# fabiocarrara/neural-ode-features

Measured on AMD Instinct MI355X. Metric: images/sec (fwd+adjoint) CIFAR-10 ODE-ResNet bs=128 at 1/2/4/8 GPU, higher is better.
Workload: dtype f32

## Files before the change

### neural-ode-features_amd/csrc/kernels_pointwise.hip

```cpp
#include "node_internal.h"
#include "wino4.h"
#include "step_control.h"
#include <cstring>
#include "../../include/node_hip.h"

namespace node {


__device__ inline float wave_sum(float v) {
#pragma unroll
  for (int off = 32; off > 0; off >>= 1) v += __shfl_xor(v, off, 64);
  return v;
}
__device__ inline float wave_max(float v) {
#pragma unroll
  for (int off = 32; off > 0; off >>= 1) v = fmaxf(v, __shfl_xor(v, off, 64));
  return v;
}

__device__ inline float block_sum_256(float v, float* red ) {
  v = wave_sum(v);
  __syncthreads();
  if ((threadIdx.x & 63) == 0) red[threadIdx.x >> 6] = v;
  __syncthreads();
// ... 801 lines not shown
}
void launch_fill(float* p, float v, size_t n, hipStream_t s) {
  size_t blocks = (n + 255) / 256;
  if (blocks > 2048) blocks = 2048;
  if (blocks == 0) return;
  hipLaunchKernelGGL(k_fill, dim3((unsigned)blocks), dim3(256), 0, s, p, v, n);
}

__global__ __launch_bounds__(256) void k_dot_partial(const float* a, const float* b, size_t n, float* partial) {
  __shared__ float red[4];
  float acc = 0.f;
  const size_t stride = (size_t)gridDim.x * 256;
  for (size_t i = (size_t)blockIdx.x * 256 + threadIdx.x; i < n; i += stride) acc += a[i] * b[i];
  const float tot = block_sum_256(acc, red);
  if (threadIdx.x == 0) partial[blockIdx.x] = tot;
}
__global__ __launch_bounds__(256) void k_dot_final(Ctrl* c, const float* partial, float sign, float* out_dot) {
  __shared__ float red[4];
  const float tot = sign * reduce_partials_512(partial, red);
  if (threadIdx.x == 0) {
    c->ts_cur = c->ts_cur - tot;
    if (out_dot) *out_dot = tot;
  }
}
void launch_dot_sub_scalar(Ctrl* ctrl, const float* a, const float* b, size_t n, float sign, float* partial, float* out_dot, hipStream_t s) {
  hipLaunchKernelGGL(k_dot_partial, dim3(ERR_BLOCKS), dim3(256), 0, s, a, b, n, partial);
  hipLaunchKernelGGL(k_dot_final, dim3(1), dim3(256), 0, s, ctrl, partial, sign, out_dot);
}
__global__ void k_copy_scalar_out(const Ctrl* c, float* dst) { *dst = c->ts_cur; }
void launch_copy_scalar_out(const Ctrl* ctrl, float* dst, hipStream_t s) {
  hipLaunchKernelGGL(k_copy_scalar_out, dim3(1), dim3(1), 0, s, ctrl, dst);
}

__global__ __launch_bounds__(256) void k_theta_finalize(ThetaFinalizeArgs a, Dims d) {
  if (a.ctrl->done) return;
  __shared__ float red[256];
  __shared__ int s_last;
  const ThetaLayout L = theta_layout(d.C);
  const int C = d.C;
  const int nsm = (9 * C + 63) / 64;
  const int bx_all = blockIdx.x;
  const int wb = ((int)gridDim.x - 5 * nsm) / 2;
  if (bx_all >= 5 * nsm) {
    const int layer = (bx_all - 5 * nsm) / wb, bx = (bx_all - 5 * nsm) - layer * wb;
    const size_t CC = (size_t)C * C;
    const size_t n4 = 9 * CC / 4;
    const float4* wp = reinterpret_cast<const float4*>(a.wpart[layer]);
    float4* out = reinterpret_cast<float4*>(a.theta_out + L.wc[layer]);
    const size_t stride = (size_t)wb * 256;
    if (a.dU != nullptr) {
      const size_t cc4 = CC / 4;
      const float4* du = reinterpret_cast<const float4*>(a.dU + (size_t)layer * W4_COMPS * CC);
      for (size_t i = (size_t)bx * 256 + threadIdx.x; i < cc4; i += stride) {
        float4 tq[6][3];
#pragma unroll
        for (int xi = 0; xi < 6; ++xi) {
          float4 u[6];
#pragma unroll
          for (int nu = 0; nu < 6; ++nu) u[nu] = du[(size_t)(xi * 6 + nu) * cc4 + i];
#pragma unroll
          for (int kw = 0; kw < 3; ++kw) {
            float4 s = make_float4(0.f, 0.f, 0.f, 0.f);
#pragma unroll
            for (int nu = 0; nu < 6; ++nu) {
              const float gq = (float)W4_G[nu][kw];
              if (gq != 0.f) { s.x += gq * u[nu].x; s.y += gq * u[nu].y; s.z += gq * u[nu].z; s.w += gq * u[nu].w; }
            }
// ... 62 lines not shown
      a.theta_out[(which ? L.b[layer] : L.g[layer]) + (col - which * C)] = a.osign * v;
    }
    return;
  }
  if (on) {
    a.theta_out[L.wt[layer] + col] = a.osign * (v * eval_time(a.et));
    if (col >= 4 * C && col < 5 * C) a.theta_out[L.cb[layer] + (col - 4 * C)] = a.osign * v;
  }
  const int nb = (9 * C + 63) / 64;
  float* dotpart = a.sred + (size_t)2 * 9 * C;
  unsigned* counter = reinterpret_cast<unsigned*>(dotpart + 2 * nb);
  const float part = wave_sum(on ? v * a.wtime[layer][col] : 0.f);
#if defined(__HIP_DEVICE_COMPILE__) && !defined(__gfx950__)
#error "k_theta_finalize's fence-free hand-off is only valid on gfx950: use release/acquire on the counter elsewhere"
#endif
  if (cl == 0) {
    __hip_atomic_store(dotpart + layer * nb + bxs, part, __ATOMIC_RELAXED, __HIP_MEMORY_SCOPE_AGENT);
    asm volatile("s_waitcnt vmcnt(0)" ::: "memory");
    s_last = __hip_atomic_fetch_add(counter, 1u, __ATOMIC_RELAXED, __HIP_MEMORY_SCOPE_AGENT) == (unsigned)(2 * nb - 1);
  }
  __builtin_amdgcn_wave_barrier();
  if (!s_last) return;
  float tot = 0.f;
  for (int i = cl; i < 2 * nb; i += 64) tot += __hip_atomic_load(dotpart + i, __ATOMIC_RELAXED, __HIP_MEMORY_SCOPE_AGENT);
  tot = wave_sum(tot);
  if (cl == 0) {
    __hip_atomic_store(counter, 0u, __ATOMIC_RELAXED, __HIP_MEMORY_SCOPE_AGENT);
    if (a.write_scalar) a.ctrl->ts_k[a.kidx] = a.osign * tot;
    if (a.vjp_t_out) *a.vjp_t_out = a.osign * tot;
  }
}

void launch_theta_finalize(const Dims& d, const ThetaFinalizeArgs& a, hipStream_t s) {
  size_t wblocks = (9 * (size_t)d.C * d.C / 4 + 255) / 256;
  if (a.dU != nullptr) wblocks = ((size_t)d.C * d.C / 4 + 255) / 256;
  if (wblocks > 1024) wblocks = 1024;
  const size_t nsmall = (9 * (size_t)d.C + 63) / 64;
  hipLaunchKernelGGL(k_theta_finalize, dim3((unsigned)(5 * nsmall + 2 * wblocks)), dim3(256), 0, s, a, d);
}

__global__ __launch_bounds__(256) void k_lincomb(Comb c, const Ctrl* ctrl, float* out, size_t n) {
  const float scale = comb_scale(c, ctrl);
  float cf[7];
#pragma unroll
  for (int j = 0; j < 7; ++j) cf[j] = scale * c.coef[j];
  const size_t stride = (size_t)gridDim.x * 256;
  for (size_t i = (size_t)blockIdx.x * 256 + threadIdx.x; i < n; i += stride) {
    float s = 0.f;
    for (int j = 0; j < c.nk; ++j) s += cf[j] * c.k[j][i];
    out[i] = c.y[i] + s;
  }
}
void launch_lincomb(const Comb& c, const Ctrl* ctrl, float* out, size_t n, hipStream_t s) {
  size_t blocks = (n + 255) / 256;
  if (blocks > 2048) blocks = 2048;
  hipLaunchKernelGGL(k_lincomb, dim3((unsigned)blocks), dim3(256), 0, s, c, ctrl, out, n);
}

}
```

### neural-ode-features_amd/csrc/node_internal.h

```cpp
#pragma once
#include <hip/hip_runtime.h>
#include <stdint.h>
#include <stddef.h>

namespace node {

constexpr int KCH = 32;
constexpr int BN = 64;
constexpr int WG_THREADS = 256;

struct Dims {
  int N, C, H, W, HW, G, cpg;
  float eps;
  int Wp, Hp, SLOTS;
  int MARGIN;
  int BNE;
  int ntile;
  int nchunk;
  int BM;
  int S;
  int wino;
  int wgrad_wino;
  int wut;
  int tiny;
// ... 323 lines not shown
void launch_pack_weights_small(const Dims& d, const float* w, float* packed , hipStream_t s);
void launch_conv_small(const Dims& d, const ConvArgs& a, hipStream_t s);

struct WgradArgs {
  const float* act;
  const float* dz;
  const Ctrl* ctrl;
  float* wpart;
  unsigned long long* stamps;
  const float* act2;
  const float* dz2;
  float* wpart2;
};
void launch_wgrad(const Dims& d, const WgradArgs& a, hipStream_t s);
size_t wgrad_lds_bytes(const Dims& d);

struct ThetaFinalizeArgs {
  const float* dU;
  const float* wpart[2];
  const float* spart[2];
  const float* gpart[3];
  int gpart_rows[3];
  int spart_rows;
  const float* wtime[2];
  float* sred;
  EvalTime et;
  float osign;
  float* theta_out;
  Ctrl* ctrl;
  int kidx;
  int write_scalar;
  float* vjp_t_out;
};
void launch_theta_finalize(const Dims& d, const ThetaFinalizeArgs& a, hipStream_t s);

struct TinyConvArgs {
  const float* act;
  const unsigned short* wq;
  const float* bias; const float* tmap;
  EvalTime et;
  const float* gamma; const float* beta;
  float* out;
  float* part; unsigned* counter;
  const Ctrl* ctrl;
  int relu; float osign;
  int nx_on, nx_self;
  Comb nx; float* nx_y_out; const float* nx_gamma; const float* nx_beta; float* nx_act;
};
struct TinyResidentArgs {
  const float* y0;
  float* y_first;
  float* y_out;
  const float* w[2];
  const float* bias[2];
  const float* gamma[3];
  const float* beta[3];
  void* handoff;
  unsigned nonce;
  Ctrl* ctrl;
  Ctrl* ctrl_host;
  const double* targets; int n_targets;
  double targets_inline[8];
  const double* forced; int n_forced;
  double* dt_log; int dt_log_cap;
  double t0;
  long long max_steps;
  float rtol, atol, tsign;
// ... 36 lines not shown
```

### neural-ode-features_amd/csrc/plan.h

```cpp
#pragma once
#include "host_common.h"
#include "wino4.h"

namespace node {

struct Plan {
  Ctrl* ctrl;
  unsigned* arrive;
  float* partial[3];
  float* wf[2];
  float* wd[2];
  float* tmap[2];
  float *Y, *Y1, *KY[7];
  float *act1, *act2;
  float* RAW;
  float* wsmall[2];
  unsigned short* wtiny[2];
  float* tpart;
  unsigned* tcount;
  void* thand;
  float *W4V, *W4M;
  float* w4u[4];
  unsigned short* w4ub[4];
  float* tmapS[2];
  W4Scales* w4sc;
  float* W4Va0b;
  float *W4Va[2], *W4Z[2], *W4dU;
  float *act1b, *xh1b, *r1b;
  float *A, *A1, *KA[7];
  float *TH, *TH1, *KT[7];
  float *xh1, *xh2, *xh3, *r1, *r2, *r3;
  float *dz1, *dz2, *G;
  float *wpart[2], *spart[2], *gpart[3], *sred, *wtime[2];
  float* dots;
  double* targets;
  double* forced;
  double* dtlog;
  size_t bytes;
};
constexpr int STEP_LIST_CAP = 4096;

Plan make_plan(const Dims& d, int adjoint, int n_t, void* base);

int check_common(const node_shape* shape, const node_params* params, void* ws, size_t ws_bytes, int adjoint, int n_t,
                 Dims* d, Plan* plan);
int check_method(int method);
int check_times(const float* t_pts, int n_t);

struct SolveCtl {
  bool forced;
  int n_forced;
  long long max_steps;
  int log_cap;
  int blind;
};
int check_solve(const node_shape* shape, const node_params* params, void* ws, size_t ws_bytes, int adjoint, const float* t_pts,
                int n_t, int method, const node_solve_opts* opts, Dims* d, Plan* plan, SolveCtl* ctl);
int solve_rc(int status, double dt);

}
```

### neural-ode-features_amd/csrc/plan.hip

```cpp
#include "plan.h"

#include <cstring>

namespace node {

Plan make_plan(const Dims& d, int adjoint, int n_t, void* base) {
  Plan p;
  memset(&p, 0, sizeof(p));
  Bump b(base);
  p.ctrl = b.take<Ctrl>(1);
  p.arrive = b.take<unsigned>(4);
  p.targets = b.take<double>((size_t)(n_t > 0 ? n_t : 1));
  p.forced = b.take<double>(STEP_LIST_CAP);
  p.dtlog = b.take<double>(STEP_LIST_CAP);
  for (int i = 0; i < 3; ++i) p.partial[i] = b.take<float>(ERR_BLOCKS * 2);
  const size_t wsz = conv_packed_elems(d);
  for (int i = 0; i < 2; ++i) p.wf[i] = b.take<float>(wsz);
  for (int i = 0; i < 2; ++i) p.tmap[i] = b.take<float>((size_t)d.HW * d.C);
  p.Y = b.take<float>(d.numel);
  p.Y1 = b.take<float>(d.numel);
  for (int i = 0; i < 7; ++i) p.KY[i] = b.take<float>(d.numel);
  p.act1 = b.take<float>(d.numel + d.C);
  p.act2 = b.take<float>(d.numel + d.C);
  if (d.csplit || d.small) p.RAW = b.take<float>(d.numel);
// ... 16 lines not shown
      for (int i = 0; i < 2; ++i) p.W4Va[i] = b.take<float>(w4_v_elems(d.N8, d.C));
      p.W4Va0b = b.take<float>(w4_v_elems(d.N8, d.C));
      for (int i = 0; i < 2; ++i) p.W4Z[i] = b.take<float>(w4_z_elems(d.N8, d.C));
      p.W4dU = b.take<float>(w4_du_elems(d.C));
    }
    if (adjoint) {
      p.act1b = b.take<float>(d.numel + d.C);
      p.xh1b = b.take<float>(d.numel);
      p.r1b = b.take<float>((size_t)d.N * d.G);
    }
  }
  const size_t prow = d.wino4 ? (size_t)d.N * d.w4q : (size_t)d.N;
  if (adjoint) {
    for (int i = 0; i < 2; ++i) p.wd[i] = b.take<float>(wsz);
    p.A = b.take<float>(d.numel);
    p.A1 = b.take<float>(d.numel);
    for (int i = 0; i < 7; ++i) p.KA[i] = b.take<float>(d.numel);
    p.TH = b.take<float>(d.P);
    p.TH1 = b.take<float>(d.P);
    for (int i = 0; i < 7; ++i) p.KT[i] = b.take<float>(d.P);
    p.xh1 = b.take<float>(d.numel);
    p.xh2 = b.take<float>(d.numel);
    p.xh3 = b.take<float>(d.numel);
    p.r1 = b.take<float>((size_t)d.N * d.G);
    p.r2 = b.take<float>((size_t)d.N * d.G);
    p.r3 = b.take<float>((size_t)d.N * d.G);
    p.dz1 = b.take<float>(d.numel + d.C);
    p.dz2 = b.take<float>(d.numel + d.C);
    p.G = b.take<float>(d.numel);
    for (int i = 0; i < 2; ++i) {
      p.wpart[i] = b.take<float>((size_t)d.nsplit * 9 * d.C * d.C);
      p.spart[i] = b.take<float>(prow * 9 * d.C);
    }
    p.sred = b.take<float>((size_t)2 * 9 * d.C + 2 * ((9 * (size_t)d.C + 63) / 64) + 4);
    for (int i = 0; i < 2; ++i) p.wtime[i] = b.take<float>((size_t)9 * d.C);
    const size_t grows = prow > (size_t)d.mtiles ? prow : (size_t)d.mtiles;
    p.gpart[0] = b.take<float>(grows * 2 * d.C);
    p.gpart[1] = b.take<float>(grows * 2 * d.C);
    p.gpart[2] = b.take<float>(prow * 2 * d.C);
    p.dots = b.take<float>((size_t)(n_t > 0 ? n_t : 1));
  }
  p.bytes = ((b.off + 255) & ~(size_t)255);
  return p;
}

int check_common(const node_shape* shape, const node_params* params, void* ws, size_t ws_bytes, int adjoint, int n_t,
                 Dims* d, Plan* plan) {
  if (!params) return fail(NODE_ERR_NULL, "params is NULL");
  if (!ws) return fail(NODE_ERR_NULL, "workspace is NULL");
  TRY(dims_for(shape, d));
  const float* ptrs[10] = {params->norm1_w, params->norm1_b, params->conv1_w, params->conv1_b, params->norm2_w,
                           params->norm2_b, params->conv2_w, params->conv2_b, params->norm3_w, params->norm3_b};
  for (int i = 0; i < 10; ++i) {
    if (!ptrs[i]) return fail(NODE_ERR_NULL, "parameter pointer %d is NULL", i);
    if (((uintptr_t)ptrs[i]) & 15) return fail(NODE_ERR_ARG, "parameter pointer %d is not 16-byte aligned", i);
  }
  if (((uintptr_t)ws) & 255) return fail(NODE_ERR_ARG, "workspace must be 256-byte aligned");
  *plan = make_plan(*d, adjoint, n_t, ws);
  if (ws_bytes < plan->bytes) return fail(NODE_ERR_WORKSPACE, "workspace too small: %zu < %zu", ws_bytes, plan->bytes);
  return NODE_OK;
}

int check_method(int method) {
  if (method != NODE_METHOD_DOPRI5 && method != NODE_METHOD_RK4) return fail(NODE_ERR_ARG, "unknown method %d", method);
  return NODE_OK;
}

int check_times(const float* t_pts, int n_t) {
  if (!t_pts) return fail(NODE_ERR_NULL, "t_pts is NULL");
  if (n_t < 2) return fail(NODE_ERR_ARG, "need at least two time points (got %d)", n_t);
  bool inc = true, dec = true;
  for (int i = 1; i < n_t; ++i) {
    if (!(t_pts[i] > t_pts[i - 1])) inc = false;
// ... 43 lines not shown
```

### neural-ode-features_amd/csrc/solver.h

```cpp
#pragma once
#include "butcher.h"
#include "plan.h"

#include <atomic>

namespace node {

struct StepGuess { int N, C, H, W, aug, forced; float rtol, atol; double t0, t1; int steps; };
int guess_steps(const StepGuess& k);
void remember_steps(const StepGuess& k);

struct SideStream;
extern int g_w4_pair_stats[4];
extern std::atomic<int> g_resident_cooldown;

struct StepIO {
  int n_targets = 0;
  int n_forced = 0;
  int log_cap = 0;
  float* y_out = nullptr;
};

struct NextComb { Comb cy; float* y_out; };

// ... 21 lines not shown
                      long long max_steps, int blind);

  bool w4_b16 = false;
  bool w4_f16 = false;
  bool w4_f16_aug = false;
  SideStream* side = nullptr;
  bool side_pending = false;
  float* va0_of(int set) const { return (set && p.W4Va0b != nullptr) ? p.W4Va0b : p.W4Va[0]; }
  bool g_ready = false;
  bool f16_now() const { return w4_f16 && (!aug || g_ready); }
  bool v_ready = false;
  int cur = 0;
  float* act1_of(int i) const { return i ? p.act1b : p.act1; }
  float* xh1_of(int i) const { return i ? p.xh1b : p.xh1; }
  float* r1_of(int i) const { return i ? p.r1b : p.r1; }
  bool w4_wgrad_on() const { return w4 && aug && p.W4dU != nullptr; }

  void to_state(const float* nchw, float* dst) {
    if (w4) launch_w4s_from_nchw(nchw, dst, d.N, d.C, d.w4q, st);
    else launch_nchw_to_nhwc(d, nchw, dst, st);
  }
  void from_state(const float* src, float* nchw) {
    if (w4) launch_w4s_to_nchw(src, nchw, d.N, d.C, d.w4q, st);
    else launch_nhwc_to_nchw(d, src, nchw, st);
  }

  void (*nr_fn)(void*, float*, int32_t, void*) = nullptr;
  void* nr_ctx = nullptr;
  float* nr_buf = nullptr;
  float nr_world = 1.f;
  void take_norm_hook(const node_solve_opts* o);
  void norm_exchange(int mode, int nseg);
  static bool fold_ctl();

  double conv_flops() const { return 2.0 * 9.0 * d.C * d.C * (double)d.N * d.HW; }
  int check_launch(const char* what);

  int prepare();

  int eval_fwd(const Comb& cy, float* y_out, const EvalTime& et, float* k_out, bool train, const NextComb* next = nullptr);
  int eval_aug(const Comb& cy, const Comb& ca, float* y_out, float* a_out, const EvalTime& et, float* kY_out, float* kA_out,
               float* kT_out, int kidx, float csign, float* vjp_t_out, bool need_theta = true, const NextComb* next = nullptr);
  int eval_sys(int kout, const double* coef, int ncoef, int scale_mode, const EvalTime& et, bool write_new, bool need_theta = true,
               const double* next_coef = nullptr, int next_ncoef = 0, bool next_write_new = false);
  EvalTime et_stage(double alpha) const { EvalTime e; e.ctrl = p.ctrl; e.alpha = (float)alpha; e.tsign = tsign; e.mode = TM_STAGE; return e; }
  EvalTime et_probe() const { EvalTime e; e.ctrl = p.ctrl; e.alpha = 0.f; e.tsign = tsign; e.mode = TM_PROBE; return e; }

  void gn_pass_fwd(const float* gamma, const float* beta, int relu, float osign, float* out, float* xhat_out, float* rstd_out);
  void gn_pass_bwd(const float* act, const float* xhat, const float* rstd, const float* gamma, float osign, float* out, float* gpart,
                   float* spart);
  void w4_gemm(int which, const float* V = nullptr);
  W4sArgs w4_args() const;
  void w4_tail_combine(W4sArgs& a, const Comb& cy, float* y_out, bool train, int set, int self);
  void w4_pass(int head, int tail, const W4sArgs& a);
  int eval_w4(const Comb& cy, float* y_out, const EvalTime& et, float* kY_out, bool train, const Comb* ca, float* a_out, float* kA_out,
              float* kT_out, int kidx, float csign, float* vjp_t_out, bool need_theta, const NextComb* next);

  int readback();
  int initial_step();
  int enqueue_step(const StepIO& io);
  int run_steps(const StepIO& io, long long max_steps, int guess, int* status);
  int upload(double* dst, const double* src, int n, double* stage);
  int rk4_interval(double t0, double t1, const float* dot_with = nullptr, float* dot_out = nullptr);
};

struct DtLog {
// ... 13 lines not shown
```

### neural-ode-features_amd/csrc/solver.hip

```cpp
#include "solver.h"

#include <cmath>
#include <cstring>
#include <mutex>
#include <utility>
#include <vector>

namespace node {

static thread_local std::vector<StepGuess> g_guess;
int guess_steps(const StepGuess& k) {
  for (const auto& g : g_guess)
    if (g.N == k.N && g.C == k.C && g.H == k.H && g.W == k.W && g.aug == k.aug && g.forced == k.forced && g.rtol == k.rtol &&
        g.atol == k.atol && g.t0 == k.t0 && g.t1 == k.t1)
      return g.steps;
  return 1;
}
void remember_steps(const StepGuess& k) {
  for (auto& g : g_guess)
    if (g.N == k.N && g.C == k.C && g.H == k.H && g.W == k.W && g.aug == k.aug && g.forced == k.forced && g.rtol == k.rtol &&
        g.atol == k.atol && g.t0 == k.t0 && g.t1 == k.t1) { g.steps = k.steps; return; }
  if (g_guess.size() >= 64) g_guess.erase(g_guess.begin());
  g_guess.push_back(k);
}
// ... 96 lines not shown
    ra.nonce = nn;
  }
  ra.targets = inline_targets ? nullptr : p.targets; ra.n_targets = io.n_targets;
  if (inline_targets) for (int j = 0; j < io.n_targets; ++j) ra.targets_inline[j] = ts[j + 1];
  ra.forced = forced ? p.forced : nullptr; ra.n_forced = io.n_forced;
  ra.dt_log = io.log_cap > 0 ? p.dtlog : nullptr; ra.dt_log_cap = io.log_cap;
  ra.t0 = ts[0]; ra.max_steps = max_steps;
  ra.rtol = rtol; ra.atol = atol; ra.tsign = tsign;
  if (!blind) { hctrl->done = 0; hctrl->status = NODE_ERR_HIP; }
  launch_tiny_solve(d, ra, st);
  nfe = forced ? 1 : 2;
  return NODE_OK;
}

void Solver::take_norm_hook(const node_solve_opts* o) {
  if (o != nullptr && o->norm_reduce != nullptr && o->norm_buf != nullptr && o->norm_world >= 1) {
    nr_fn = o->norm_reduce; nr_ctx = o->norm_reduce_ctx; nr_buf = o->norm_buf; nr_world = (float)o->norm_world;
  }
}

void Solver::norm_exchange(int mode, int nseg) {
  NormPackArgs np;
  memset(&np, 0, sizeof(np));
  np.ctrl = p.ctrl; np.partial[0] = p.partial[0]; np.partial[1] = p.partial[1]; np.partial[2] = p.partial[2];
  np.nseg = nseg; np.has_scalar = aug ? 1 : 0; np.mode = mode; np.rtol = rtol; np.atol = atol;
  np.w4sc = (aug && w4_f16) ? p.w4sc : nullptr; np.gbuf = nr_buf;
  launch_norm_pack(np, st);
  nr_fn(nr_ctx, nr_buf, 8, (void*)st);
}

bool Solver::fold_ctl() {
  return env_int("NODE_TUNE_FOLD_CTL", 0) != 0;
}

int Solver::check_launch(const char* what) {
  hipError_t e = hipGetLastError();
  if (e != hipSuccess) return fail(NODE_ERR_HIP, "launch of %s failed: %s", what, hipGetErrorString(e));
  return NODE_OK;
}

int Solver::prepare() {
  auto pack = d.wino == 2 ? launch_pack_weights_w2 : d.wino ? launch_pack_weights_w : launch_pack_weights;
  float* zr[12];
  size_t zn[12];
  int nz = 0;
  zr[nz] = reinterpret_cast<float*>(p.arrive); zn[nz++] = 4;
  if (aug) {
    zr[nz] = p.KT[1]; zn[nz++] = d.P;
    zr[nz] = p.sred + (size_t)2 * 9 * d.C + 2 * ((9 * (size_t)d.C + 63) / 64); zn[nz++] = 1;
  }
  if (d.wino == 2 || d.wgrad_wino == 2 || small_mode()) {
    zr[nz] = p.act1 + d.numel; zn[nz++] = d.C;
    zr[nz] = p.act2 + d.numel; zn[nz++] = d.C;
    if (aug) {
      zr[nz] = p.dz1 + d.numel; zn[nz++] = d.C;
      zr[nz] = p.dz2 + d.numel; zn[nz++] = d.C;
      if (p.act1b) { zr[nz] = p.act1b + d.numel; zn[nz++] = d.C; }
    }
  }
  if (small_mode()) {
    launch_pack_weights_small(d, prm.conv1_w, p.wsmall[0], st);
    launch_pack_weights_small(d, prm.conv2_w, p.wsmall[1], st);
  }
  if (tiny_mode() && !w4) {
    launch_tiny_pack(d, prm.conv1_w, p.wtiny[0], st);
    launch_tiny_pack(d, prm.conv2_w, p.wtiny[1], st);
    launch_fill(reinterpret_cast<float*>(p.tcount), 0.f, (size_t)d.N * d.G, st);
  }
  if (w4) {
    w4_b16 = w4_uses_bf16(d.N8, d.C);
    w4_f16 = w4_b16 && w4_f16_fits(d.N8, d.C) && (!aug || (w4_f16_aug && w4_wgrad_on() && w4_wgrad_f16_fits(d.N8, d.C)));
    g_ready = false;
    side = nullptr; side_pending = false;
    if (w4_f16 && aug) {
      if (env_int("NODE_TUNE_W4_WGRAD_SIDE", 0) != 0 && !get_side(&side)) side = nullptr;
    }
    if (w4_f16) { zr[nz] = reinterpret_cast<float*>(p.w4sc); zn[nz++] = sizeof(W4Scales) / sizeof(float); }
  }
  launch_time_prep(d, prm.conv1_w, prm.conv2_w, p.tmap[0], p.tmap[1], aug ? p.wtime[0] : nullptr, aug ? p.wtime[1] : nullptr, zr, zn,
                   nz, st);
  if (w4) {
    W4PackJobs jobs;
// ... 6 lines not shown
      sj.gb[0] = prm.norm1_w; sj.gb[1] = prm.norm1_b; sj.gb[2] = prm.norm2_w; sj.gb[3] = prm.norm2_b;
      sj.C = d.C; sj.gn_m = d.cpg * d.HW; sj.sc = p.w4sc;
      launch_w4_scales(sj, st);
    }
    for (int i = 0; i < (aug ? 4 : 2); ++i) {
      jobs.w[i] = ws_[i]; jobs.u[i] = p.w4u[i]; jobs.dgrad[i] = i >= 2;
      if (w4_f16) { jobs.uh[i] = reinterpret_cast<unsigned*>(p.w4u[i]); jobs.uh_exp[i] = &p.w4sc->e[(i & 1) ? W4_E_U2 : W4_E_U1]; }
      if (!w4_f16 || aug) jobs.ub[i] = w4_b16 ? p.w4ub[i] : nullptr;
    }
    launch_w4_pack(jobs, aug ? 4 : 2, d.C, st);
  } else if (d.wino == 2) {
    const float* ws_[4] = {prm.conv1_w, prm.conv2_w, prm.conv1_w, prm.conv2_w};
    float* dst_[4] = {p.wf[0], p.wf[1], p.wd[0], p.wd[1]};
    const int dg_[4] = {0, 0, 1, 1};
    launch_pack_weights_w2_multi(d, ws_, dst_, dg_, aug ? 4 : 2, st);
  } else {
    pack(d, prm.conv1_w, p.wf[0], 0, st);
    pack(d, prm.conv2_w, p.wf[1], 0, st);
    if (aug) {
      pack(d, prm.conv1_w, p.wd[0], 1, st);
      pack(d, prm.conv2_w, p.wd[1], 1, st);
    }
  }
  if (w4) launch_w4s_tmap(p.tmap[0], p.tmap[1], p.tmapS[0], p.tmapS[1], d.C, d.w4q, st);
  if (w4 && aug && d.N * d.w4q != d.N8 && p.W4dU != nullptr) {
    for (int i = 0; i < 2; ++i) {
      launch_fill(p.W4Va[i], 0.f, w4_v_elems(d.N8, d.C), st);
      launch_fill(p.W4Z[i], 0.f, w4_z_elems(d.N8, d.C), st);
    }
    launch_fill(p.W4Va0b, 0.f, w4_v_elems(d.N8, d.C), st);
  }
  v_ready = false;
  cur = 0;
  return check_launch("prepare");
}

void Solver::gn_pass_fwd(const float* gamma, const float* beta, int relu, float osign, float* out, float* xhat_out, float* rstd_out) {
  CombineGnArgs ca;
  memset(&ca, 0, sizeof(ca));
  ca.comb.y = p.RAW; ca.comb.nk = 0; ca.comb.scale_mode = SC_ABS; ca.ctrl = p.ctrl;
  ca.act_out = out; ca.xhat_out = xhat_out; ca.rstd_out = rstd_out;
  ca.gamma = gamma; ca.beta = beta; ca.relu = relu; ca.osign = osign;
  launch_combine_gn(d, ca, st);
}
void Solver::gn_pass_bwd(const float* act, const float* xhat, const float* rstd, const float* gamma, float osign, float* out,
                 float* gpart, float* spart) {
  GnBwdArgs g;
  memset(&g, 0, sizeof(g));
  g.comb.y = p.RAW; g.comb.nk = 0; g.comb.scale_mode = SC_ABS; g.ctrl = p.ctrl; g.csign = 1.f;
  g.xhat = xhat; g.rstd = rstd; g.gamma = gamma; g.dz_out = out; g.gpart = gpart; g.spart = spart;
  g.mask_act = act; g.osign = osign;
  launch_gn_bwd(d, g, st);
}

void Solver::w4_gemm(int which, const float* V) {
  ProfScope ps(2, conv_flops(), st);
  if (f16_now()) {
    launch_w4_gemm_f16(reinterpret_cast<const unsigned*>(V ? V : p.W4V), reinterpret_cast<const unsigned*>(p.w4u[which]), p.W4M, p.ctrl, d.N8, d.C,
                       &p.w4sc->e[which >= 2 ? W4_E_G : which ? W4_E_V2 : W4_E_V1], &p.w4sc->e[(which & 1) ? W4_E_U2 : W4_E_U1], st);
    return;
  }
  launch_w4_gemm(V ? V : p.W4V, p.w4u[which], p.W4M, p.ctrl, d.N8, d.C, st, w4_b16 ? p.w4ub[which] : nullptr);
}

W4sArgs Solver::w4_args() const {
  W4sArgs a;
// ... 14 lines not shown
  if (g_prof.on) {
    const double state = (double)d.numel * sizeof(float), comp = 36.0 * 4.0 * d.N * d.w4q * d.C * sizeof(float);
    int tensors = 0;
    if (head) {
      tensors += (a.h.out_s != nullptr) + (a.h.out_nhwc != nullptr);
      tensors += a.h.xhat_s != nullptr;
      bytes += comp;
    }
    if (tail) {
      tensors += 1 + a.t.comb.nk - (a.t.self ? 1 : 0);
      tensors += (a.t.y_out != nullptr) + (a.t.act_nhwc != nullptr) + (a.t.xhat_s != nullptr);
    }
    if (a.V) bytes += comp;
    bytes += tensors * state;
  }
  const int cls = head == 0 ? 3 : head == 1 ? 4 + tail : 7 + tail;
  ProfScope ps(cls, bytes, st);
  launch_w4s_pass(head, tail, a, st);
}

int Solver::eval_w4(const Comb& cy, float* y_out, const EvalTime& et, float* kY_out, bool train, const Comb* ca, float* a_out,
            float* kA_out, float* kT_out, int kidx, float csign, float* vjp_t_out, bool need_theta, const NextComb* next) {
  const bool do_aug = ca != nullptr;
  if (next != nullptr)
    for (int j = 0; j + 1 < next->cy.nk; ++j)
      if (next->cy.k[j] == kY_out || (do_aug && next->cy.k[j] == kA_out)) next = nullptr;
  if (!v_ready) {
    W4sArgs a = w4_args();
    w4_tail_combine(a, cy, y_out, train, cur, 0);
    w4_pass(0, 1, a);
  }
  v_ready = false;
  const bool wg4 = do_aug && w4_wgrad_on();
  w4_gemm(0, wg4 ? va0_of(cur) : nullptr);
  {
    W4sArgs a = w4_args();
    a.h.M = p.W4M; a.h.bias = prm.conv1_b; a.h.tmapS = p.tmapS[0]; a.h.et = et; a.h.gamma = prm.norm2_w; a.h.beta = prm.norm2_b;
    a.h.osign = 1.f; a.h.relu = 1;
    if (train) { a.h.out_nhwc = wg4 ? nullptr : p.act2; a.h.xhat_s = p.xh2; a.h.rstd = p.r2; }
    a.V = wg4 ? p.W4Va[1] : p.W4V;
    if (f16_now()) a.v_exp = &p.w4sc->e[W4_E_V2];
    w4_pass(1, 0, a);
  }
  w4_gemm(1, wg4 ? p.W4Va[1] : nullptr);
  W4sArgs a3 = w4_args();
  a3.h.M = p.W4M; a3.h.bias = prm.conv2_b; a3.h.tmapS = p.tmapS[1]; a3.h.et = et; a3.h.gamma = prm.norm3_w; a3.h.beta = prm.norm3_b;
  a3.h.osign = et.tsign; a3.h.relu = 0; a3.h.out_s = kY_out;
  if (!do_aug) {
    if (next != nullptr) {
      const int self = next->cy.nk > 0 && next->cy.k[next->cy.nk - 1] == kY_out;
      w4_tail_combine(a3, next->cy, next->y_out, false, cur, self);
      w4_pass(1, 1, a3);
      v_ready = true;
    } else {
      w4_pass(1, 0, a3);
    }
    if (count_nfe) nfe += 1;
    return check_launch("odefunc forward (F(4x4,3x3))");
  }
  a3.t.comb = *ca; a3.t.csign = csign; a3.t.y_out = a_out; a3.t.gpart = p.gpart[2]; a3.t.spart = p.spart[1];
  if (wg4) a3.t.z_out = need_theta ? p.W4Z[1] : nullptr;
  else a3.t.act_nhwc = p.dz2;
  a3.V = p.W4V;
  if (w4_f16) a3.gstat = p.w4sc;
  if (f16_now()) { a3.v_exp = &p.w4sc->e[W4_E_G]; a3.z_exp = &p.w4sc->e[W4_E_G]; }
  w4_pass(1, 2, a3);
  if (count_nfe) nfe += 1;
  w4_gemm(3);
  {
    W4sArgs a = w4_args();
    a.h.M = p.W4M; a.h.gamma = prm.norm2_w; a.h.beta = prm.norm2_b; a.h.xhat_s = p.xh2; a.h.rstd = p.r2; a.h.osign = 1.f;
    a.h.gpart = p.gpart[1]; a.h.spart = p.spart[0];
    if (wg4) a.h.z_out = need_theta ? p.W4Z[0] : nullptr;
    else a.h.out_nhwc = p.dz1;
    a.V = p.W4V;
    if (w4_f16) a.gstat = p.w4sc;
    if (f16_now()) { a.v_exp = &p.w4sc->e[W4_E_G]; a.z_exp = &p.w4sc->e[W4_E_G]; }
    w4_pass(2, 0, a);
  }
  if (need_theta && wg4 && f16_now()) {
    hipStream_t ws = st;
    if (side != nullptr) {
      (void)hipEventRecord(side->fork, st);
      (void)hipStreamWaitEvent(side->s, side->fork, 0);
      ws = side->s;
    }
    {
      ProfScope ps(1, 2.0 * conv_flops(), ws);
      launch_w4_wgrad_f16(reinterpret_cast<const unsigned*>(va0_of(cur)), reinterpret_cast<const unsigned*>(p.W4Z[0]), reinterpret_cast<const unsigned*>(p.W4Va[1]),
                          reinterpret_cast<const unsigned*>(p.W4Z[1]), p.W4dU, p.ctrl, d.N8, d.C, &p.w4sc->e[W4_E_V1], &p.w4sc->e[W4_E_V2], &p.w4sc->e[W4_E_G], ws);
    }
    if (side != nullptr) { (void)hipEventRecord(side->join, side->s); side_pending = true; }
  } else if (need_theta && wg4) {
    W4WgradArgs wa;
    memset(&wa, 0, sizeof(wa));
    wa.V1 = va0_of(cur); wa.Z1 = p.W4Z[0]; wa.V2 = p.W4Va[1]; wa.Z2 = p.W4Z[1]; wa.dU = p.W4dU; wa.ctrl = p.ctrl; wa.N = d.N8; wa.C = d.C;
    ProfScope ps(1, 2.0 * conv_flops(), st);
    launch_w4_wgrad(wa, st);
  } else if (need_theta) {
    WgradArgs w1;
    memset(&w1, 0, sizeof(w1));
    w1.act = act1_of(cur); w1.dz = p.dz1; w1.wpart = p.wpart[0]; w1.ctrl = p.ctrl;
    if (d.wgrad_pair) { w1.act2 = p.act2; w1.dz2 = p.dz2; w1.wpart2 = p.wpart[1]; }
    { ProfScope ps(1, (d.wgrad_pair ? 2.0 : 1.0) * conv_flops(), st); launch_wgrad(d, w1, st); }
    if (!d.wgrad_pair) {
      WgradArgs w2 = w1;
      w2.act = p.act2; w2.dz = p.dz2; w2.wpart = p.wpart[1];
      { ProfScope ps(1, conv_flops(), st); launch_wgrad(d, w2, st); }
    }
  }
  w4_gemm(2);
  {
    W4sArgs a = w4_args();
    a.h.M = p.W4M; a.h.gamma = prm.norm1_w; a.h.beta = prm.norm1_b; a.h.xhat_s = xh1_of(cur); a.h.rstd = r1_of(cur);
    a.h.osign = et.tsign; a.h.out_s = kA_out; a.h.gpart = p.gpart[0];
    if (next != nullptr) {
      w4_tail_combine(a, next->cy, next->y_out, true, cur ^ 1, 0);
      w4_pass(2, 1, a);
      cur ^= 1;
      v_ready = true;
    } else {
      w4_pass(2, 0, a);
    }
  }
  if (!need_theta) return check_launch("augmented dynamics (F(4x4,3x3))");
  if (side_pending) { (void)hipStreamWaitEvent(st, side->join, 0); side_pending = false; }
  ThetaFinalizeArgs tf;
  memset(&tf, 0, sizeof(tf));
  tf.dU = wg4 ? p.W4dU : nullptr;
  tf.wpart[0] = p.wpart[0]; tf.wpart[1] = p.wpart[1];
  tf.spart[0] = p.spart[0]; tf.spart[1] = p.spart[1];
  tf.gpart[0] = p.gpart[0]; tf.gpart[1] = p.gpart[1]; tf.gpart[2] = p.gpart[2];
  tf.gpart_rows[0] = tf.gpart_rows[1] = tf.gpart_rows[2] = tf.spart_rows = d.N * d.w4q;
  tf.wtime[0] = p.wtime[0]; tf.wtime[1] = p.wtime[1]; tf.sred = p.sred;
  tf.et = et; tf.osign = et.tsign; tf.theta_out = kT_out;
  tf.ctrl = p.ctrl; tf.kidx = kidx; tf.write_scalar = kidx >= 0 ? 1 : 0; tf.vjp_t_out = vjp_t_out;
  launch_theta_finalize(d, tf, st);
  return check_launch("augmented dynamics (F(4x4,3x3))");
}

int Solver::eval_fwd(const Comb& cy, float* y_out, const EvalTime& et, float* k_out, bool train, const NextComb* next) {
  if (w4) return eval_w4(cy, y_out, et, k_out, train, nullptr, nullptr, nullptr, nullptr, -1, 0.f, nullptr, false, next);
  const bool tiny = tiny_mode() && !train;
  if (!(tiny && v_ready)) {
    CombineGnArgs ca;
    memset(&ca, 0, sizeof(ca));
    ca.comb = cy; ca.ctrl = p.ctrl; ca.y_out = y_out; ca.act_out = p.act1;
    ca.xhat_out = train ? p.xh1 : nullptr; ca.rstd_out = train ? p.r1 : nullptr;
    ca.gamma = prm.norm1_w; ca.beta = prm.norm1_b; ca.relu = 1; ca.osign = 1.f;
    launch_combine_gn(d, ca, st);
  }
  v_ready = false;

  if (tiny) {
    TinyConvArgs t1;
    memset(&t1, 0, sizeof(t1));
    t1.act = p.act1; t1.wq = p.wtiny[0]; t1.bias = prm.conv1_b; t1.tmap = p.tmap[0]; t1.et = et;
    t1.gamma = prm.norm2_w; t1.beta = prm.norm2_b; t1.out = p.act2; t1.part = p.tpart; t1.counter = p.tcount; t1.ctrl = p.ctrl;
    t1.relu = 1; t1.osign = 1.f;
    { ProfScope ps(0, conv_flops(), st); launch_tiny_conv_gn(d, t1, st); }
    TinyConvArgs t2 = t1;
    t2.act = p.act2; t2.wq = p.wtiny[1]; t2.bias = prm.conv2_b; t2.tmap = p.tmap[1];
    t2.gamma = prm.norm3_w; t2.beta = prm.norm3_b; t2.out = k_out; t2.relu = 0; t2.osign = et.tsign;
    if (next != nullptr) {
      t2.nx_on = 1; t2.nx = next->cy; t2.nx_self = -1;
      for (int j = 0; j < next->cy.nk; ++j)
        if (next->cy.k[j] == k_out) t2.nx_self = j;
      t2.nx_y_out = next->y_out; t2.nx_gamma = prm.norm1_w; t2.nx_beta = prm.norm1_b; t2.nx_act = p.act1;
      v_ready = true;
    }
// ... 109 lines not shown
}

int Solver::initial_step() {
  const int nseg = aug ? 3 : 1;
  InitSeg segs[3] = {{p.Y, p.KY[0], p.KY[1], d.numel}, {p.A, p.KA[0], p.KA[1], d.numel}, {p.TH, p.KT[0], p.KT[1], d.P}};
  InitCtlArgs ic;
  memset(&ic, 0, sizeof(ic));
  ic.ctrl = p.ctrl;
  for (int i = 0; i < nseg; ++i) { ic.partial[i] = p.partial[i]; ic.numel[i] = (double)segs[i].n; }
  ic.nseg = nseg; ic.has_scalar = aug ? 1 : 0; ic.phase = 0; ic.rtol = rtol; ic.atol = atol;
  const bool fold = nr_fn == nullptr && fold_ctl();
  if (fold) launch_init_norms_ctl(segs, p.partial, nseg, ic, p.arrive, st);
  else {
    launch_init_norms(segs, p.partial, nseg, rtol, atol, 0, st);
    if (nr_fn != nullptr) { norm_exchange(1, nseg); ic.gbuf = nr_buf; ic.gworld = nr_world; }
    launch_init_controller(ic, st);
  }
  const double one[1] = {1.0};
  TRY(eval_sys(1, one, 1, SC_H0, et_probe(), false));
  ic.phase = 1;
  if (fold) launch_init_norms_ctl(segs, p.partial, nseg, ic, p.arrive, st);
  else {
    launch_init_norms(segs, p.partial, nseg, rtol, atol, 1, st);
    if (nr_fn != nullptr) norm_exchange(2, nseg);
    launch_init_controller(ic, st);
  }
  return check_launch("initial step");
}

int Solver::enqueue_step(const StepIO& io) {
  static const int skip_k2 = env_int("NODE_TUNE_SKIP_K2_THETA", 1);
  const bool was_counting = count_nfe;
  count_nfe = false;
  for (int s = 0; s < 6; ++s) {
    const int rc = eval_sys(s + 1, DP_BETA[s], s + 1, SC_DT, et_stage(DP_ALPHA[s]), s == 5, !(skip_k2 && s == 0),
                            s < 5 ? DP_BETA[s + 1] : nullptr, s + 2, s + 1 == 5);
    if (rc != NODE_OK) { count_nfe = was_counting; return rc; }
  }
  count_nfe = was_counting;
  const int nseg = aug ? 3 : 1;
  ErrSeg es[3];
  es[0].y0 = p.Y; es[0].y1 = p.Y1; es[0].n = d.numel; es[0].compute_y1 = 0;
  for (int j = 0; j < 7; ++j) es[0].k[j] = p.KY[j];
  if (aug) {
    es[1] = es[0];
    es[1].y0 = p.A; es[1].y1 = p.A1;
    for (int j = 0; j < 7; ++j) es[1].k[j] = p.KA[j];
    es[2].y0 = p.TH; es[2].y1 = p.TH1; es[2].n = d.P; es[2].compute_y1 = 1;
    for (int j = 0; j < 7; ++j) es[2].k[j] = p.KT[j];
  }
  StepCtlArgs sc;
  memset(&sc, 0, sizeof(sc));
  sc.ctrl = p.ctrl;
  sc.partial[0] = p.partial[0]; sc.partial[1] = p.partial[1]; sc.partial[2] = p.partial[2];
  sc.numel[0] = (double)d.numel; sc.numel[1] = (double)d.numel; sc.numel[2] = (double)d.P;
  sc.nseg = nseg; sc.has_scalar = aug ? 1 : 0; sc.rtol = rtol; sc.atol = atol;
  sc.targets = p.targets; sc.n_targets = io.n_targets;
  sc.forced = io.n_forced > 0 ? p.forced : nullptr; sc.n_forced = io.n_forced;
  sc.dt_log = io.log_cap > 0 ? p.dtlog : nullptr; sc.dt_log_cap = io.log_cap;
  sc.interp_scalar = aug ? 1 : 0;
  sc.w4sc = (aug && w4_f16) ? p.w4sc : nullptr;
  if (nr_fn == nullptr && fold_ctl()) {
    launch_error_norm_ctl(es, p.partial, nseg, sc, p.arrive, st);
  } else {
    launch_error_norm(es, p.partial, nseg, p.ctrl, rtol, atol, st);
    if (nr_fn != nullptr) { norm_exchange(0, nseg); sc.gbuf = nr_buf; sc.gworld = nr_world; }
    launch_step_controller(sc, st);
  }
  if (!aug) {
    EmitArgs ea;
    ea.ctrl = p.ctrl; ea.targets = p.targets; ea.y0 = p.Y; ea.y1 = p.Y1;
    for (int j = 0; j < 7; ++j) ea.k[j] = p.KY[j];
// ... 63 lines not shown
```

Baseline: 28250.

## Batch per-stage theta finalize into one launch per Dormand-Prince step

Theta-gradient finalization for stages 2-6 of each adaptive step is now deferred into a single batched launch instead of five. Each stage writes its partials into its own slot buffers (dU, spart, gpart, sred), and blockIdx.y picks the slot. The goal is fewer small kernel launches and less serialization, plus a wider grid for the finalize work. The cost is extra workspace for per-slot buffers. Correctness now depends on nothing consuming a stage's theta output or scalar before the step ends.

```diff
diff --git a/neural-ode-features_amd/csrc/kernels_pointwise.hip b/neural-ode-features_amd/csrc/kernels_pointwise.hip
--- a/neural-ode-features_amd/csrc/kernels_pointwise.hip
+++ b/neural-ode-features_amd/csrc/kernels_pointwise.hip
@@ -857,7 +857,8 @@
   hipLaunchKernelGGL(k_copy_scalar_out, dim3(1), dim3(1), 0, s, ctrl, dst);
 }
 
-__global__ __launch_bounds__(256) void k_theta_finalize(ThetaFinalizeArgs a, Dims d) {
+__global__ __launch_bounds__(256) void k_theta_finalize(ThetaFinalizeBatch b, Dims d) {
+  const ThetaFinalizeArgs& a = b.st[blockIdx.y];
   if (a.ctrl->done) return;
   __shared__ float red[256];
   __shared__ int s_last;
@@ -986,11 +987,19 @@
 }
 
 void launch_theta_finalize(const Dims& d, const ThetaFinalizeArgs& a, hipStream_t s) {
+  ThetaFinalizeBatch b;
+  memset(&b, 0, sizeof(b));
+  b.st[0] = a; b.n = 1;
+  launch_theta_finalize_batch(d, b, s);
+}
+void launch_theta_finalize_batch(const Dims& d, const ThetaFinalizeBatch& b, hipStream_t s) {
+  if (b.n <= 0) return;
+  const ThetaFinalizeArgs& a = b.st[0];
   size_t wblocks = (9 * (size_t)d.C * d.C / 4 + 255) / 256;
   if (a.dU != nullptr) wblocks = ((size_t)d.C * d.C / 4 + 255) / 256;
   if (wblocks > 1024) wblocks = 1024;
   const size_t nsmall = (9 * (size_t)d.C + 63) / 64;
-  hipLaunchKernelGGL(k_theta_finalize, dim3((unsigned)(5 * nsmall + 2 * wblocks)), dim3(256), 0, s, a, d);
+  hipLaunchKernelGGL(k_theta_finalize, dim3((unsigned)(5 * nsmall + 2 * wblocks), (unsigned)b.n), dim3(256), 0, s, b, d);
 }
 
 __global__ __launch_bounds__(256) void k_lincomb(Comb c, const Ctrl* ctrl, float* out, size_t n) {
diff --git a/neural-ode-features_amd/csrc/node_internal.h b/neural-ode-features_amd/csrc/node_internal.h
--- a/neural-ode-features_amd/csrc/node_internal.h
+++ b/neural-ode-features_amd/csrc/node_internal.h
@@ -379,7 +379,11 @@
   int write_scalar;
   float* vjp_t_out;
 };
+__host__ __device__ inline size_t theta_sred_elems(int C) { return (((size_t)2 * 9 * C + 2 * ((9 * (size_t)C + 63) / 64) + 4) + 63) & ~(size_t)63; }
+constexpr int THETA_SLOTS = 5;
+struct ThetaFinalizeBatch { ThetaFinalizeArgs st[THETA_SLOTS]; int n; };
 void launch_theta_finalize(const Dims& d, const ThetaFinalizeArgs& a, hipStream_t s);
+void launch_theta_finalize_batch(const Dims& d, const ThetaFinalizeBatch& b, hipStream_t s);
 
 struct TinyConvArgs {
   const float* act;
diff --git a/neural-ode-features_amd/csrc/plan.h b/neural-ode-features_amd/csrc/plan.h
--- a/neural-ode-features_amd/csrc/plan.h
+++ b/neural-ode-features_amd/csrc/plan.h
@@ -33,6 +33,7 @@
   float *dz1, *dz2, *G;
   float *wpart[2], *spart[2], *gpart[3], *sred, *wtime[2];
   float* dots;
+  float *th_dU[THETA_SLOTS], *th_spart[THETA_SLOTS][2], *th_gpart[THETA_SLOTS][3], *th_sred[THETA_SLOTS];
   double* targets;
   double* forced;
   double* dtlog;
diff --git a/neural-ode-features_amd/csrc/plan.hip b/neural-ode-features_amd/csrc/plan.hip
--- a/neural-ode-features_amd/csrc/plan.hip
+++ b/neural-ode-features_amd/csrc/plan.hip
@@ -72,13 +72,23 @@
       p.wpart[i] = b.take<float>((size_t)d.nsplit * 9 * d.C * d.C);
       p.spart[i] = b.take<float>(prow * 9 * d.C);
     }
-    p.sred = b.take<float>((size_t)2 * 9 * d.C + 2 * ((9 * (size_t)d.C + 63) / 64) + 4);
+    p.sred = b.take<float>(theta_sred_elems(d.C));
     for (int i = 0; i < 2; ++i) p.wtime[i] = b.take<float>((size_t)9 * d.C);
     const size_t grows = prow > (size_t)d.mtiles ? prow : (size_t)d.mtiles;
     p.gpart[0] = b.take<float>(grows * 2 * d.C);
     p.gpart[1] = b.take<float>(grows * 2 * d.C);
     p.gpart[2] = b.take<float>(prow * 2 * d.C);
     p.dots = b.take<float>((size_t)(n_t > 0 ? n_t : 1));
+    if (d.wino4 && d.C % 128 == 0) {
+      const size_t nsred = theta_sred_elems(d.C);
+      float* sredx = b.take<float>((THETA_SLOTS - 1) * nsred);
+      for (int s = 0; s < THETA_SLOTS; ++s) {
+        p.th_dU[s] = s ? b.take<float>(w4_du_elems(d.C)) : p.W4dU;
+        for (int i = 0; i < 2; ++i) p.th_spart[s][i] = s ? b.take<float>(prow * 9 * d.C) : p.spart[i];
+        for (int i = 0; i < 3; ++i) p.th_gpart[s][i] = s ? b.take<float>(prow * 2 * d.C) : p.gpart[i];
+        p.th_sred[s] = s ? (sredx != nullptr ? sredx + (size_t)(s - 1) * nsred : nullptr) : p.sred;
+      }
+    }
   }
   p.bytes = ((b.off + 255) & ~(size_t)255);
   return p;
diff --git a/neural-ode-features_amd/csrc/solver.h b/neural-ode-features_amd/csrc/solver.h
--- a/neural-ode-features_amd/csrc/solver.h
+++ b/neural-ode-features_amd/csrc/solver.h
@@ -77,6 +77,9 @@
   void take_norm_hook(const node_solve_opts* o);
   void norm_exchange(int mode, int nseg);
   static bool fold_ctl();
+  static bool batch_theta();
+  int th_slot = -1;
+  ThetaFinalizeBatch th_batch;
 
   double conv_flops() const { return 2.0 * 9.0 * d.C * d.C * (double)d.N * d.HW; }
   int check_launch(const char* what);
diff --git a/neural-ode-features_amd/csrc/solver.hip b/neural-ode-features_amd/csrc/solver.hip
--- a/neural-ode-features_amd/csrc/solver.hip
+++ b/neural-ode-features_amd/csrc/solver.hip
@@ -152,6 +152,9 @@
 bool Solver::fold_ctl() {
   return env_int("NODE_TUNE_FOLD_CTL", 0) != 0;
 }
+bool Solver::batch_theta() {
+  return env_int("NODE_TUNE_BATCH_THETA", 1) != 0;
+}
 
 int Solver::check_launch(const char* what) {
   hipError_t e = hipGetLastError();
@@ -168,6 +171,7 @@
   if (aug) {
     zr[nz] = p.KT[1]; zn[nz++] = d.P;
     zr[nz] = p.sred + (size_t)2 * 9 * d.C + 2 * ((9 * (size_t)d.C + 63) / 64); zn[nz++] = 1;
+    if (p.W4dU != nullptr) { zr[nz] = p.th_sred[1]; zn[nz++] = (THETA_SLOTS - 1) * theta_sred_elems(d.C); }
   }
   if (d.wino == 2 || d.wgrad_wino == 2 || small_mode()) {
     zr[nz] = p.act1 + d.numel; zn[nz++] = d.C;
@@ -240,6 +244,7 @@
   }
   v_ready = false;
   cur = 0;
+  th_slot = -1;
   return check_launch("prepare");
 }
 
@@ -320,6 +325,11 @@
   }
   v_ready = false;
   const bool wg4 = do_aug && w4_wgrad_on();
+  const bool th_later = wg4 && need_theta && th_slot >= 0;
+  const int ts = th_later ? th_slot : 0;
+  float* const dU = wg4 ? p.th_dU[ts] : p.W4dU;
+  float* const gp[3] = {wg4 ? p.th_gpart[ts][0] : p.gpart[0], wg4 ? p.th_gpart[ts][1] : p.gpart[1], wg4 ? p.th_gpart[ts][2] : p.gpart[2]};
+  float* const sp[2] = {wg4 ? p.th_spart[ts][0] : p.spart[0], wg4 ? p.th_spart[ts][1] : p.spart[1]};
   w4_gemm(0, wg4 ? va0_of(cur) : nullptr);
   {
     W4sArgs a = w4_args();
@@ -346,7 +356,7 @@
     if (count_nfe) nfe += 1;
     return check_launch("odefunc forward (F(4x4,3x3))");
   }
-  a3.t.comb = *ca; a3.t.csign = csign; a3.t.y_out = a_out; a3.t.gpart = p.gpart[2]; a3.t.spart = p.spart[1];
+  a3.t.comb = *ca; a3.t.csign = csign; a3.t.y_out = a_out; a3.t.gpart = gp[2]; a3.t.spart = sp[1];
   if (wg4) a3.t.z_out = need_theta ? p.W4Z[1] : nullptr;
   else a3.t.act_nhwc = p.dz2;
   a3.V = p.W4V;
@@ -358,7 +368,7 @@
   {
     W4sArgs a = w4_args();
     a.h.M = p.W4M; a.h.gamma = prm.norm2_w; a.h.beta = prm.norm2_b; a.h.xhat_s = p.xh2; a.h.rstd = p.r2; a.h.osign = 1.f;
-    a.h.gpart = p.gpart[1]; a.h.spart = p.spart[0];
+    a.h.gpart = gp[1]; a.h.spart = sp[0];
     if (wg4) a.h.z_out = need_theta ? p.W4Z[0] : nullptr;
     else a.h.out_nhwc = p.dz1;
     a.V = p.W4V;
@@ -376,13 +386,13 @@
     {
       ProfScope ps(1, 2.0 * conv_flops(), ws);
       launch_w4_wgrad_f16(reinterpret_cast<const unsigned*>(va0_of(cur)), reinterpret_cast<const unsigned*>(p.W4Z[0]), reinterpret_cast<const unsigned*>(p.W4Va[1]),
-                          reinterpret_cast<const unsigned*>(p.W4Z[1]), p.W4dU, p.ctrl, d.N8, d.C, &p.w4sc->e[W4_E_V1], &p.w4sc->e[W4_E_V2], &p.w4sc->e[W4_E_G], ws);
+                          reinterpret_cast<const unsigned*>(p.W4Z[1]), dU, p.ctrl, d.N8, d.C, &p.w4sc->e[W4_E_V1], &p.w4sc->e[W4_E_V2], &p.w4sc->e[W4_E_G], ws);
     }
     if (side != nullptr) { (void)hipEventRecord(side->join, side->s); side_pending = true; }
   } else if (need_theta && wg4) {
     W4WgradArgs wa;
     memset(&wa, 0, sizeof(wa));
-    wa.V1 = va0_of(cur); wa.Z1 = p.W4Z[0]; wa.V2 = p.W4Va[1]; wa.Z2 = p.W4Z[1]; wa.dU = p.W4dU; wa.ctrl = p.ctrl; wa.N = d.N8; wa.C = d.C;
+    wa.V1 = va0_of(cur); wa.Z1 = p.W4Z[0]; wa.V2 = p.W4Va[1]; wa.Z2 = p.W4Z[1]; wa.dU = dU; wa.ctrl = p.ctrl; wa.N = d.N8; wa.C = d.C;
     ProfScope ps(1, 2.0 * conv_flops(), st);
     launch_w4_wgrad(wa, st);
   } else if (need_theta) {
@@ -401,7 +411,7 @@
   {
     W4sArgs a = w4_args();
     a.h.M = p.W4M; a.h.gamma = prm.norm1_w; a.h.beta = prm.norm1_b; a.h.xhat_s = xh1_of(cur); a.h.rstd = r1_of(cur);
-    a.h.osign = et.tsign; a.h.out_s = kA_out; a.h.gpart = p.gpart[0];
+    a.h.osign = et.tsign; a.h.out_s = kA_out; a.h.gpart = gp[0];
     if (next != nullptr) {
       w4_tail_combine(a, next->cy, next->y_out, true, cur ^ 1, 0);
       w4_pass(2, 1, a);
@@ -415,15 +425,16 @@
   if (side_pending) { (void)hipStreamWaitEvent(st, side->join, 0); side_pending = false; }
   ThetaFinalizeArgs tf;
   memset(&tf, 0, sizeof(tf));
-  tf.dU = wg4 ? p.W4dU : nullptr;
+  tf.dU = wg4 ? dU : nullptr;
   tf.wpart[0] = p.wpart[0]; tf.wpart[1] = p.wpart[1];
-  tf.spart[0] = p.spart[0]; tf.spart[1] = p.spart[1];
-  tf.gpart[0] = p.gpart[0]; tf.gpart[1] = p.gpart[1]; tf.gpart[2] = p.gpart[2];
+  tf.spart[0] = sp[0]; tf.spart[1] = sp[1];
+  tf.gpart[0] = gp[0]; tf.gpart[1] = gp[1]; tf.gpart[2] = gp[2];
   tf.gpart_rows[0] = tf.gpart_rows[1] = tf.gpart_rows[2] = tf.spart_rows = d.N * d.w4q;
-  tf.wtime[0] = p.wtime[0]; tf.wtime[1] = p.wtime[1]; tf.sred = p.sred;
+  tf.wtime[0] = p.wtime[0]; tf.wtime[1] = p.wtime[1]; tf.sred = th_later ? p.th_sred[ts] : p.sred;
   tf.et = et; tf.osign = et.tsign; tf.theta_out = kT_out;
   tf.ctrl = p.ctrl; tf.kidx = kidx; tf.write_scalar = kidx >= 0 ? 1 : 0; tf.vjp_t_out = vjp_t_out;
-  launch_theta_finalize(d, tf, st);
+  if (th_later) th_batch.st[ts] = tf;
+  else launch_theta_finalize(d, tf, st);
   return check_launch("augmented dynamics (F(4x4,3x3))");
 }
 
@@ -599,12 +610,20 @@
   static const int skip_k2 = env_int("NODE_TUNE_SKIP_K2_THETA", 1);
   const bool was_counting = count_nfe;
   count_nfe = false;
+  const bool th_batched = aug && w4_wgrad_on() && batch_theta();
+  if (th_batched) memset(&th_batch, 0, sizeof(th_batch));
   for (int s = 0; s < 6; ++s) {
+    th_slot = (th_batched && s >= 1) ? s - 1 : -1;
     const int rc = eval_sys(s + 1, DP_BETA[s], s + 1, SC_DT, et_stage(DP_ALPHA[s]), s == 5, !(skip_k2 && s == 0),
                             s < 5 ? DP_BETA[s + 1] : nullptr, s + 2, s + 1 == 5);
-    if (rc != NODE_OK) { count_nfe = was_counting; return rc; }
-  }
+    if (rc != NODE_OK) { count_nfe = was_counting; th_slot = -1; return rc; }
+  }
+  th_slot = -1;
   count_nfe = was_counting;
+  if (th_batched) {
+    th_batch.n = THETA_SLOTS;
+    launch_theta_finalize_batch(d, th_batch, st);
+  }
   const int nseg = aug ? 3 : 1;
   ErrSeg es[3];
   es[0].y0 = p.Y; es[0].y1 = p.Y1; es[0].n = d.numel; es[0].compute_y1 = 0;
```

Result: no change. 28470, median of 6 (+0.8%).
